# sclaus2/CutFEMx

Measured on AMD Instinct MI355X. Metric: assembled DOFs/sec (active dofs / full hot-path step) + cut-quadrature points/sec, Poisson P1 sphere level-set, higher is better.
Workload: dtype f64; 1 GPU; 3D Poisson P1, sphere level set on 512^3 background mesh (805306368 tets), Nitsche + ghost penalty, runtime quadrature order 4; one step = cut + rules + sparsity + assemble_matrix + assemble_vector + deactivation; cells=805306368, active_dofs=17125633, parallelism=1 gpu

## Files before the change

### cutfemx_amd/csrc/cfx_device.h

```cpp
#pragma once

#include "cfx_common.h"

namespace cfx
{

constexpr int kBlock = 256;
constexpr int kScanItems = 8;
constexpr int kTile = kBlock * kScanItems;

__device__ __forceinline__ int64_t xcd_block_id()
{
  const int64_t per = gridDim.x >> 3;
  return (int64_t)(blockIdx.x & 7) * per + (blockIdx.x >> 3);
}

inline dim3 xcd_grid(int64_t nblocks)
{
  const int64_t g = (nblocks + 7) / 8 * 8;
  if (g > 2147483647LL) throw Error(CFX_ERR_RUNTIME, "grid too large");
  return dim3((unsigned)g);
}

__device__ __forceinline__ void block_fill_run(double* __restrict__ p, int n, double v)
{
  const int head = (int)((reinterpret_cast<uintptr_t>(p) >> 3) & 1) & (n > 0 ? 1 : 0);
  if (threadIdx.x == 0 && head) p[0] = v;
  const int npair = (n - head) >> 1;
  double2* q = reinterpret_cast<double2*>(p + head);
  const double2 vv = make_double2(v, v);
  for (int k = threadIdx.x; k < npair; k += blockDim.x) q[k] = vv;
  if (threadIdx.x == 0 && ((n - head) & 1)) p[n - 1] = v;
}

__host__ __device__ __forceinline__ uint32_t cfx_hash32(uint32_t h)
{
  h ^= h >> 16; h *= 0x85ebca6bu;
  h ^= h >> 13; h *= 0xc2b2ae35u;
  h ^= h >> 16;
  return h;
}

constexpr int kAdjPer = 4, kAdjRun = kBlock * kAdjPer, kAdjSlots = 2 * kAdjRun;
__device__ __forceinline__ int adj_lds_insert(int32_t* s_key, int32_t* s_cnt, int32_t item, int& rank)
{
  unsigned h = cfx_hash32((uint32_t)item) & (kAdjSlots - 1);
  for (;;)
  {
    const int32_t prev = atomicCAS(&s_key[h], -1, item);
    if (prev == -1 || prev == item) break;
    h = (h + 1) & (kAdjSlots - 1);
  }
  rank = atomicAdd(&s_cnt[h], 1);
  return (int)h;
}

template <typename T>
__device__ __forceinline__ T wave_inclusive_scan(T v)
{
  const int lane = threadIdx.x & 63;
#pragma unroll
  for (int d = 1; d < 64; d <<= 1)
  {
    T up = __shfl_up(v, d, 64);
    if (lane >= d) v += up;
  }
  return v;
}

template <typename T>
__device__ __forceinline__ T block_exclusive_scan(T v, T& total)
{
  __shared__ T wave_sums[kBlock / 64];
  const int lane = threadIdx.x & 63, wave = threadIdx.x >> 6;
  T incl = wave_inclusive_scan(v);
  __syncthreads();
  if (lane == 63) wave_sums[wave] = incl;
  __syncthreads();
  T base = 0, tot = 0;
#pragma unroll
  for (int w = 0; w < kBlock / 64; ++w)
  {
    T s = wave_sums[w];
    if (w < wave) base += s;
    tot += s;
  }
  total = tot;
  return base + incl - v;
}

constexpr int kChainLook = 4;
constexpr unsigned long long kScanAggregate = 1ull << 62, kScanPrefix = 2ull << 62, kScanValueMask = (1ull << 62) - 1ull;

struct ChainState
{
  unsigned long long* state = nullptr;
  unsigned int* ticket = nullptr;
};
ChainState chain_state(int64_t ntiles);
inline ChainState fused_chain(bool publish, int64_t ntiles)
{
  const int64_t max_tiles = env_int_once<Sw::FUSED_TILES>(512);
  return publish && ntiles <= max_tiles ? chain_state(ntiles) : ChainState{};
}

__device__ __forceinline__ unsigned int chain_take_tile(unsigned int* __restrict__ ticket)
{
  __shared__ unsigned int s_tile;
  if (threadIdx.x == 0) s_tile = atomicAdd(ticket, 1u);
  __syncthreads();
  return s_tile;
}

__device__ __forceinline__ unsigned long long chain_exclusive_prefix(unsigned long long* __restrict__ state,
                                                                     const unsigned int tile, const unsigned long long total)
// ... 534 lines not shown
```

### cutfemx_amd/csrc/cfx_fem.hip

```cpp
#include <cstdlib>

#include "cfx_elem.h"

using namespace cfx;

namespace
{

struct AsmArgs
{
  const double* x;
  const int32_t* conn;
  const int32_t* dofmap;
  DevN n;
  const int32_t* entities;
  const int32_t* offsets;
  const int32_t* parent_map;
  const double* points;
  const double* weights;
  const double* point_data;
  int point_stride;
  int kernel;
  int qdegree;
  double params[8];
// ... 1114 lines not shown
    }
    return;
  }
  if (!single || !use_rule)
  {
    A.n = single ? 1 : I.n_entities.value();
    A.entities = I.entities.p + (single ? only_index : 0);
    if (A.n.cap > 0)
    {
      if (tdim == 2) launch("assemble_cells2_std", assemble_cells2_kernel<2, false>, grid_for(A.n.cap * nloc0), dim3(kBlock), 0, A, R);
      else launch("assemble_cells2_std", assemble_cells2_kernel<3, false>, grid_for(A.n.cap * nloc0), dim3(kBlock), 0, A, R);
    }
  }
  if (I.rules && (!single || use_rule))
  {
    const cfx_rules_s* Q = I.rules;
    A.n = single ? 1 : Q->nr.value();
    A.offsets = Q->offsets.p + (single ? only_index : 0);
    A.parent_map = Q->parent_map.p + (single ? only_index : 0);
    A.points = Q->points.p; A.weights = Q->weights.p;
    if (A.n.cap > 0)
    {
      if (tdim == 2) launch("assemble_cells2_cut", assemble_cells2_kernel<2, true>, grid_for(A.n.cap * nloc0), dim3(kBlock), 0, A, R);
      else launch("assemble_cells2_cut", assemble_cells2_kernel<3, true>, grid_for(A.n.cap * nloc0), dim3(kBlock), 0, A, R);
    }
  }
}

__global__ void mark_cells_kernel(DevN n_d, const int32_t* __restrict__ cells, int stride, uint8_t* mark)
{
  const int64_t n = dev_n(n_d);
  const int64_t i = (int64_t)blockIdx.x * blockDim.x + threadIdx.x;
  if (i < n) mark[cells[i * stride]] = 1;
}

__global__ void mark_dofs_kernel(int64_t ncells_active, const int32_t* __restrict__ cells,
                                 const int32_t* __restrict__ dofmap, int nd, int bs, uint8_t* indicator)
{
  const int64_t i = (int64_t)blockIdx.x * blockDim.x + threadIdx.x;
  if (i >= ncells_active * nd) return;
  const int64_t c = cells[i / nd];
  const int32_t dof = dofmap[c * nd + (int)(i % nd)];
  for (int k = 0; k < bs; ++k) indicator[(int64_t)dof * bs + k] = 1;
}

bool force_atomic()
{
  return env_equals<Sw::ASSEMBLY>("atomic");
}

struct FlagSet
{
  const uint8_t* f;
  __device__ bool operator()(int64_t i) const { return f[i] != 0; }
};
struct FlagClear
{
  const uint8_t* f;
  __device__ bool operator()(int64_t i) const { return f[i] == 0; }
};

__global__ void deactivate_kernel(DevN n_d, const int32_t* __restrict__ rows, const int64_t* __restrict__ indptr,
                                  const int32_t* __restrict__ indices, double* values, double* b, double diagonal,
                                  double rhs_value, int* error)
{
  const int64_t n = dev_n(n_d);
  const int64_t i = (int64_t)blockIdx.x * blockDim.x + threadIdx.x;
  if (i >= n) return;
  const int32_t r = rows[i];
  if (values)
  {
    const int64_t rb = indptr[r], re = indptr[r + 1];
    const int64_t pos = (re - rb == 1 && indices[rb] == r) ? rb : csr_find(indices, rb, re, r);
    if (pos < 0) *error = 1; else values[pos] = diagonal;
  }
  if (b) b[r] = rhs_value;
}

__global__ void __launch_bounds__(kBlock) deactivate_marks_kernel(int64_t nrows, const uint8_t* __restrict__ rowmark,
                                                                  const int64_t* __restrict__ tile_counts,
                                                                  const int64_t* __restrict__ indptr,
                                                                  const int32_t* __restrict__ indices, double* __restrict__ values,
                                                                  double* __restrict__ b, double diagonal, double rhs_value, int* error,
                                                                  DevN n_active_d, DevN nnz_d)
{
  if (n_active_d.dev && dev_n(n_active_d) == 0) return;
  if (nnz_d.dev && dev_n(nnz_d) == 0) return;
  const int64_t r0 = (int64_t)blockIdx.x * kByteTile;
  const int tl = (int)min((int64_t)kByteTile, nrows - r0);
  const int64_t tc = tile_counts[blockIdx.x];
  const int nact = (int)((tc & 0xffffffffll) + (tc >> 32));
  if (nact == 0 && (!values || indptr[r0 + tl] - indptr[r0] == tl))
  {
    int ok = 1;
    const int64_t e0 = values ? indptr[r0] : 0;
    if (values)
      for (int k = threadIdx.x; k < tl; k += kBlock) ok &= indices[e0 + k] == (int32_t)(r0 + k) ? 1 : 0;
    if (__syncthreads_and(ok))
    {
      if (values) block_fill_run(values + e0, tl, diagonal);
      if (b) block_fill_run(b + r0, tl, rhs_value);
      return;
    }
  }
  if (nact == tl) return;
  for (int k = threadIdx.x; k < tl; k += kBlock)
  {
    const int64_t r = r0 + k;
    if (rowmark[r]) continue;
    if (values)
    {
      const int64_t rb = indptr[r], re = indptr[r + 1];
      const int64_t pos = (re - rb == 1 && indices[rb] == r) ? rb : csr_find(indices, rb, re, (int32_t)r);
      if (pos < 0) *error = 1; else values[pos] = diagonal;
    }
    if (b) b[r] = rhs_value;
  }
}

__global__ void inactive_tile_counts_kernel(int64_t ntiles, int64_t n, const int64_t* __restrict__ active, int32_t* __restrict__ zeros)
{
  const int64_t t = (int64_t)blockIdx.x * blockDim.x + threadIdx.x;
  if (t >= ntiles) return;
  const int64_t len = min((int64_t)kByteTile, n - t * kByteTile);
  zeros[t] = (int32_t)(len - (active[t] & 0xffffffffll) - (active[t] >> 32));
}

__global__ void facet_cells_covered_kernel(DevN nf_d, const int32_t* __restrict__ rows, const uint8_t* __restrict__ cellmark,
                                           int* uncovered)
{
  const int64_t nf = dev_n(nf_d);
  const int64_t i = (int64_t)blockIdx.x * blockDim.x + threadIdx.x;
  if (i >= 2 * nf) return;
  if (cellmark[rows[4 * (i >> 1) + 2 * (i & 1)]] == 0) atomicOr(uncovered, 1);
}

void collect_cell_marks(const cfx_form_s* a, bool include_facets, DevArray<uint8_t>& mark, bool& any)
{
  const int64_t nc = a->V->mesh->ncells;
  mark.alloc(nc);
  mark.zero();
  any = false;
  for (const auto& I : a->integrals)
  {
    if (I.type == CFX_CELL)
    {
      if (I.n_entities.cap() > 0)
      {
        launch("mark_cells", mark_cells_kernel, grid_for(I.n_entities.cap()), dim3(kBlock), 0, I.n_entities, I.entities.p, 1,
               mark.p);
        any = true;
      }
      if (I.rules && I.rules->nr.cap() > 0)
      {
        launch("mark_cells", mark_cells_kernel, grid_for(I.rules->nr.cap()), dim3(kBlock), 0, I.rules->nr,
               I.rules->parent_map.p, 1, mark.p);
        any = true;
      }
    }
    else if (include_facets && I.type == CFX_INTERIOR_FACET && I.n_entities.cap() > 0)
    {
      launch("mark_cells", mark_cells_kernel, grid_for(I.n_entities.cap()), dim3(kBlock), 0, I.n_entities, I.entities.p, 4,
             mark.p);
      launch("mark_cells", mark_cells_kernel, grid_for(I.n_entities.cap()), dim3(kBlock), 0, I.n_entities,
             I.entities.p + 2, 4, mark.p);
      any = true;
    }
  }
}

}

namespace
{
template <int TDIM>
__global__ void __launch_bounds__(kBlock) facet_jump_p1_kernel(DevN n_d, const int32_t* __restrict__ rows,
                                                               const double* __restrict__ x, const int32_t* __restrict__ conn,
                                                               const int32_t* __restrict__ dofmap, double gamma, double hpow,
                                                               int qdegree, double* __restrict__ out, int* error)
{
  const int64_t n = dev_n(n_d);
  constexpr int ND = TDIM + 1;
  const int64_t f = (int64_t)blockIdx.x * kBlock + threadIdx.x;
  if (f >= n) return;
  const int4 row4 = *reinterpret_cast<const int4*>(rows + 4 * f);
  const int64_t c0 = row4.x, c1 = row4.z;
  const int lf0 = row4.y;
  Geo<TDIM> g0, g1;
  load_cell<TDIM>(x, conn, c0, g0);
  load_cell<TDIM>(x, conn, c1, g1);
  jacobian<TDIM>(g0);
  jacobian<TDIM>(g1);
  const double havg = 0.5 * (cell_diameter<TDIM>(g0) + cell_diameter<TDIM>(g1));
  double nrm[TDIM], nn = 0.0;
#pragma unroll
  for (int d = 0; d < TDIM; ++d)
  {
    double v = 0.0;
#pragma unroll
    for (int t = 0; t < TDIM; ++t) v -= g0.K[t][d] * ((lf0 == 0) ? -1.0 : ((lf0 - 1 == t) ? 1.0 : 0.0));
// ... 1230 lines not shown
  cfx_row_plan& plan = *d->plan;
  const int64_t nc = V->mesh->ncells;
  const uint8_t* cell_ind = plan.cellmark.p;
  if (plan.nfacets.value() > 0 && !plan.facet_rows.owned)
  {
    for (const auto& k : plan.key_facets)
      if (k[1] == (int64_t)(uintptr_t)plan.facet_rows.p && k[5] != 0 && dev_block_serial(plan.facet_rows.p) != (uint64_t)k[5])
        throw Error(CFX_ERR_RUNTIME, "stale active domain: the facet list of the form it was made from was released; ask for "
                                     "the lists while the form is alive (the Python wrapper keeps it)");
  }
  if (plan.nfacets.value() > 0)
  {
    ZeroFlag uncovered;
    const int64_t nf = plan.nfacets.value();
    launch("active_cells", facet_cells_covered_kernel, grid_for(nf * 2), dim3(kBlock), 0, nf, plan.facet_rows.p,
           plan.cellmark.p, uncovered.p);
    if (read_scalar(uncovered.p))
    {
      d->cell_indicator.alloc((nc + 3) & ~3LL);
      CFX_HIP(hipMemcpyAsync(d->cell_indicator.p, plan.cellmark.p, (size_t)nc, hipMemcpyDeviceToDevice, ctx().stream));
      launch("mark_cells", mark_cells_kernel, grid_for(nf), dim3(kBlock), 0, nf, plan.facet_rows.p, 4, d->cell_indicator.p);
      launch("mark_cells", mark_cells_kernel, grid_for(nf), dim3(kBlock), 0, nf, plan.facet_rows.p + 2, 4, d->cell_indicator.p);
      cell_ind = d->cell_indicator.p;
    }
  }
  const int32_t* known_tiles = (cell_ind == plan.cellmark.p && plan.cell_tile_counts.n == (nc + kByteTile - 1) / kByteTile)
                                   ? plan.cell_tile_counts.p : nullptr;
  d->n_active = Count(compact_bytes("active_cells", nc, cell_ind, ByteNonZero{}, d->active_cells, known_tiles));
  const int64_t nrows = V->ndofs * V->bs;
  if (V->bs == 1)
    d->n_inactive = Count(compact_bytes("inactive_dofs", nrows, plan.rowmark.p, ByteZero{}, d->inactive_dofs, nullptr,
                                        nrows - plan.n_active_rows.value()));
  else
  {
    DevArray<uint8_t> ind(nrows);
    ind.zero();
    const int64_t nact = d->n_active.value();
    launch("mark_dofs", mark_dofs_kernel, grid_for(nact * V->ndofs_cell), dim3(kBlock), 0, nact,
           d->active_cells.p, V->dofmap.p, V->ndofs_cell, V->bs, ind.p);
    d->n_inactive = Count(compact_bytes("inactive_dofs", nrows, ind.p, ByteZero{}, d->inactive_dofs));
  }
  d->lists_built = true;
}
}

extern "C" {

int cfx_active_view(cfx_active_t d, const int32_t** active_cells, int64_t* n_active, const int32_t** inactive_dofs,
                    int64_t* n_inactive)
{
  CFX_API_BEGIN
  require(d != nullptr, CFX_ERR_INVALID_ARGUMENT, "cfx_active_view: null handle");
  if (!active_cells && !n_active && !inactive_dofs)
  {
    if (n_inactive) *n_inactive = d->V->ndofs * d->V->bs - d->plan->n_active_rows.cap() * d->V->bs;
    return CFX_OK;
  }
  active_lists(d);
  if (active_cells) *active_cells = d->active_cells.p;
  if (n_active) *n_active = d->n_active.cap();
  if (inactive_dofs) *inactive_dofs = d->inactive_dofs.p;
  if (n_inactive) *n_inactive = d->n_inactive.cap();
  CFX_API_END
}

int cfx_deactivate_outside(cfx_active_t d, cfx_pattern_t P, double* values, double* b, double diagonal,
                           double rhs_value)
{
  CFX_API_BEGIN
  require(d && (values == nullptr || P), CFX_ERR_INVALID_ARGUMENT, "cfx_deactivate_outside: null argument");
  const int64_t nrows = d->V->ndofs * d->V->bs;
  std::unique_ptr<OutArray<double>> ov, ob;
  if (values) ov = std::make_unique<OutArray<double>>(values, count_for_buffer(P->nnz, values), true);
  if (b) ob = std::make_unique<OutArray<double>>(b, nrows, true);
  const char* kNoDiag = "Deactivated matrix row has no diagonal entry.";
  ErrorFlag err(CFX_ERR_RUNTIME, kNoDiag);
  cfx_row_plan& plan = *d->plan;
  const int64_t ntiles = (nrows + kByteTile - 1) / kByteTile;
  if (d->V->bs == 1 && plan.row_tile_counts.n == ntiles && (!values || P->nrows == nrows))
  {
    launch("deactivate", deactivate_marks_kernel, dim3((unsigned)ntiles), dim3(kBlock), 0, nrows, plan.rowmark.p,
           plan.row_tile_counts.p, values ? P->indptr.p : (const int64_t*)nullptr, values ? P->indices.p : (const int32_t*)nullptr,
           values ? ov->dev : (double*)nullptr, b ? ob->dev : (double*)nullptr, diagonal, rhs_value, err.p,
           plan.n_active_rows.devn(), values ? P->nnz.devn() : DevN());
  }
  else
  {
    active_lists(d);
    const int64_t n_inactive = d->n_inactive.value();
    if (n_inactive > 0)
      launch("deactivate", deactivate_kernel, grid_for(n_inactive), dim3(kBlock), 0, n_inactive,
             d->inactive_dofs.p, P ? P->indptr.p : nullptr, P ? P->indices.p : nullptr, values ? ov->dev : nullptr,
             b ? ob->dev : nullptr, diagonal, rhs_value, err.p);
  }
  err.check(CFX_ERR_RUNTIME, kNoDiag);
  if (ov) ov->finish();
  if (ob) ob->finish();
  CFX_API_END
}

int cfx_active_destroy(cfx_active_t d)
{
  CFX_API_BEGIN
  delete d;
  CFX_API_END
}

}
```

### cutfemx_amd/csrc/cfx_gather.hip

```cpp
#include <cstdlib>
#include <type_traits>

#include "cfx_elem.h"

using namespace cfx;

namespace cfx
{
void dump_integral(cfx_form_s* a, int integral, int parts, double* out, bool fold_facets = false);
void dump_facet_jumps_p1(cfx_form_s* a, int integral, double* out, int* error);
void dump_facet_jumps_p2(cfx_form_s* a, int integral, int nq, double* out);
void dump_cut_moments(cfx_form_s* a, int integral, double* out);
int quad_npoints(int dim, int degree);
}

namespace
{

constexpr int kWave = 64;
#ifndef CFX_XCD_TILE
#define CFX_XCD_TILE 128
#endif
__device__ __forceinline__ int64_t row_block_id(int64_t b)
{
// ... 2844 lines not shown
        }
    }
    constexpr int W = 2 * NLOC;
    const double* T = A.facet_tensors + f * (int64_t)(W * W);
#pragma unroll
    for (int side = 0; side < 2; ++side)
    {
      double acc[NLOC];
      int csl[ND];
#pragma unroll
      for (int j = 0; j < NLOC; ++j) acc[j] = 0.0;
#pragma unroll
      for (int j = 0; j < ND; ++j) csl[j] = -1;
      if (has)
      {
#pragma unroll
        for (int m = 0; m < 2; ++m)
          if (irow[m] >= 0)
          {
            const double* Tr = T + (int64_t)(irow[m] * BS + kc) * W + side * NLOC;
#pragma unroll
            for (int j = 0; j < NLOC; ++j) acc[j] += Tr[j];
          }
#pragma unroll
        for (int j = 0; j < ND; ++j) csl[j] = find_slot(cols[side][j]);
#pragma unroll
        for (int j = 0; j < ND; ++j)
#pragma unroll
          for (int b = 0; b < BS; ++b)
            if (row_bc || (A.bc1 != nullptr && A.bc1[(int64_t)cols[side][j] * BS + b] != 0)) acc[j * BS + b] = 0.0;
      }
      if constexpr (ORDERED)
      {
        for (int turn = 0; turn < G; ++turn)
        {
          if (gl == turn)
          {
#pragma unroll
            for (int j = 0; j < ND; ++j)
              if (csl[j] >= 0)
              {
#pragma unroll
                for (int b = 0; b < BS; ++b) s_val[grp][csl[j] * BS + b] += acc[j * BS + b];
              }
          }
          __syncthreads();
        }
      }
      else
      {
#pragma unroll
        for (int j = 0; j < ND; ++j)
          if (csl[j] >= 0)
          {
#pragma unroll
            for (int b = 0; b < BS; ++b) atomicAdd(&s_val[grp][csl[j] * BS + b], acc[j * BS + b]);
          }
      }
    }
  }
  __syncthreads();
  if (A.fresh)
    for (int k = gl; k < lene; k += G) A.values[rb + k] = s_val[grp][k];
  else
    for (int k = gl; k < lene; k += G) A.values[rb + k] += s_val[grp][k];
}

__global__ void __launch_bounds__(kBlock) zero_inactive_rows_kernel(int64_t nrows, int bs, const uint8_t* __restrict__ rowmark,
                                                                    const int64_t* __restrict__ indptr, double* __restrict__ values,
                                                                    DevN nnz_d)
{
  const int64_t nnz = dev_n(nnz_d);
  const int64_t R = (int64_t)blockIdx.x * kBlock + threadIdx.x;
  if (R >= nrows || nnz == 0 || rowmark[R / bs]) return;
  const int64_t e1 = min(indptr[R + 1], nnz);
  for (int64_t k = max(indptr[R], (int64_t)0); k < e1; ++k) values[k] = 0.0;
}

__global__ void __launch_bounds__(kBlock) zero_inactive_tiles_kernel(int64_t nrows, const uint8_t* __restrict__ rowmark,
                                                                     const int64_t* __restrict__ tile_counts,
                                                                     const int64_t* __restrict__ indptr, double* __restrict__ values,
                                                                     DevN nnz_d)
{
  const int64_t nnz = dev_n(nnz_d);
  if (nnz == 0) return;
  const int64_t r0 = (int64_t)blockIdx.x * kByteTile;
  const int n = (int)min((int64_t)kByteTile, nrows - r0);
  if (tile_counts[blockIdx.x] == 0)
  {
    const int64_t e0 = indptr[r0];
    if (e0 >= 0 && e0 + n <= nnz) block_fill_run(values + e0, n, 0.0);
    return;
  }
  for (int k = threadIdx.x; k < n; k += kBlock)
    if (!rowmark[r0 + k])
    {
      const int64_t e1 = min(indptr[r0 + k + 1], nnz);
      for (int64_t e = max(indptr[r0 + k], (int64_t)0); e < e1; ++e) values[e] = 0.0;
    }
}

template <int TDIM, int DEG, int G>
__global__ void __launch_bounds__(kWave) assemble_vec_rows_kernel(RowArgs A)
{
  constexpr int ND = Elem<TDIM, DEG>::ND;
  constexpr int RPW = kWave / G;
  const int lane = threadIdx.x, grp = lane / G, gl = lane % G;
  const int64_t ri = CFX_ROW_BLOCK * RPW + grp;
  if (A.vec_skip && dev_n(A.vec_n_odd) == 0) return;
  bool live = ri < dev_n(A.n_active) && A.cellmark != nullptr;
  const int64_t r = live ? A.active_rows[ri] : 0;
  if (live && A.vec_skip && A.vec_skip[r] > 0) live = false;
  const int64_t cb = live ? A.d2c_off[r] : 0;
  const int nc = live ? (int)(A.d2c_off[r + 1] - cb) : 0;
  double part = 0.0;
  const unsigned dpos = (live && A.slot4) ? (A.diagpos[r] & kDiagPosMask) : 0u;
  constexpr int R = G <= 4 ? 6 : 4;
  for (int base = 0;; base += R * G)
  {
    if (__ballot(base + gl < nc) == 0) break;
    int64_t cell[R];
    uint8_t mk[R];
    int lr[R];
    uint32_t s4[R];
#pragma unroll
    for (int k = 0; k < R; ++k)
    {
      const int t = base + k * G + gl;
      cell[k] = t < nc ? (int64_t)A.d2c[cb + t] : -1;
      s4[k] = (A.slot4 && t < nc) ? A.slot4[cb + t] : 0u;
      if (DEG == 2 && A.slotn && t < nc) s4[k] = reinterpret_cast<const uint32_t*>(A.slotn + (cb + t) * 12)[2];
    }
#pragma unroll
    for (int k = 0; k < R; ++k) mk[k] = cell[k] >= 0 ? A.cellmark[cell[k]] : (uint8_t)0;
#pragma unroll
    for (int k = 0; k < R; ++k)
    {
      lr[k] = 0;
      if (!mk[k]) continue;
      if (DEG == 2 && A.slotn) lr[k] = (int)((s4[k] >> 16) & 0xffu);
      else if (A.slot4)
      {
#pragma unroll
        for (int j = 0; j < ND; ++j) lr[k] = (((s4[k] >> (8 * j)) & 0xffu) == dpos) ? j : lr[k];
      }
      else
      {
#pragma unroll
        for (int j = 0; j < ND; ++j) lr[k] = (A.dofmap[cell[k] * ND + j] == (int32_t)r) ? j : lr[k];
      }
    }
#pragma unroll
    for (int k = 0; k < R; ++k)
    {
      if (!mk[k]) continue;
      const int64_t c = cell[k];
      for (int i = 0; i < A.n_cell; ++i)
      {
        const RowIntegral& I = A.cell[i];
        if ((mk[k] & (1u << i)) && I.std_tensors)
          part += I.std_tensors[(int64_t)lr[k] * I.n_std + (I.std_by_cell ? c : entity_index(I.std_bits, I.std_rank, c))];
        if (mk[k] & (16u << i))
          for (int64_t e = first_rule(I.rule_keys, I.rule_first, I.rule_mask, (int32_t)c); e < dev_len(I.nr) && I.parent_map[e] == c; ++e)
            part += I.rule_tensors[e * ND + lr[k]];
      }
    }
  }
#pragma unroll
  for (int d = G / 2; d >= 1; d >>= 1) part += __shfl_xor(part, d, G);
  if (live && gl == 0) A.values[r] += part;
}

bool deterministic()
{
  return env_is<Sw::DETERMINISTIC>('1');
}

struct P2PlainArgs
{
  int64_t n;
  const int32_t* rows;
  const double* x;
// ... 2051 lines not shown
```

### cutfemx_amd/csrc/cfx_rowasm.hip

```cpp
#include <cmath>
#include <cstdlib>


#include "cfx_elem.h"

using namespace cfx;

namespace
{

constexpr int kWave = 64;

__global__ void plan_mark_cells_kernel(DevN n_d, const int32_t* __restrict__ cells, int stride, uint8_t bit,
                                       uint8_t* mark)
{
  const int64_t n = dev_n(n_d);
  const int64_t i = (int64_t)blockIdx.x * blockDim.x + threadIdx.x;
  if (i >= n) return;
  const int64_t c = cells[i * stride];
  mark[c] = mark[c] | bit;
}

__global__ void __launch_bounds__(kBlock) plan_pack_bits_kernel(int64_t ncells, const uint8_t* __restrict__ mark, uint8_t bit,
                                                                unsigned long long* __restrict__ words,
// ... 916 lines not shown
        const int4 q4 = l4[m];
        rank += (q4.x < v ? 1 : 0) + (q4.y < v ? 1 : 0) + (q4.z < v ? 1 : 0) + (q4.w < v ? 1 : 0);
      }
      if (P.indices)
      {
        const int bc = P.bs_col ? P.bs_col : P.bs;
        for (int a = 0; a < P.bs; ++a)
          for (int b = 0; b < bc; ++b)
            P.indices[P.indptr[r * P.bs + a] + (int64_t)rank * bc + b] = v * bc + b;
      }
      else
        P.tmp[ri * T + rank] = v;
    }
  if (cnt >= T) *P.overflow = 1;
  if (live && gl == 0 && !P.indices)
  {
    if (cnt > *reinterpret_cast<volatile int*>(P.maxlen)) atomicMax(P.maxlen, cnt);
    P.len[ri] = cnt;
    for (int a = 0; a < P.bs; ++a) P.counts[r * P.bs + a] = cnt * (P.bs_col ? P.bs_col : P.bs);
  }
  __syncthreads();
  }
}

__global__ void fill_i32_kernel(int64_t n, int32_t v, int32_t* out)
{
  const int64_t i = (int64_t)blockIdx.x * blockDim.x + threadIdx.x;
  if (i < n) out[i] = v;
}

__global__ void pattern_diag_kernel(int64_t ndofs, int bs, const uint8_t* __restrict__ rowmark,
                                    const int64_t* __restrict__ indptr, int32_t* __restrict__ indices)
{
  const int64_t r = (int64_t)blockIdx.x * blockDim.x + threadIdx.x;
  if (r >= ndofs || rowmark[r]) return;
  for (int a = 0; a < bs; ++a)
    for (int b = 0; b < bs; ++b) indices[indptr[r * bs + a] + b] = (int32_t)(r * bs + b);
}

__global__ void __launch_bounds__(kBlock) indptr_reduce_kernel(int64_t nrows, int bs, const uint8_t* __restrict__ rowmark,
                                                               const int32_t* __restrict__ counts, int64_t* __restrict__ tile_sums)
{
  const int64_t tile = (int64_t)blockIdx.x * kTile;
  int64_t s = 0;
  if (bs == 1 && tile + kTile <= nrows)
  {
    static_assert(kScanItems == 8, "eight rows per thread");
    const int64_t r0 = tile + 8 * threadIdx.x;
    const uint2 m = *reinterpret_cast<const uint2*>(rowmark + r0);
    if ((m.x | m.y) == 0u) s = 8;
    else
    {
#pragma unroll
      for (int q = 0; q < 8; ++q)
      {
        const unsigned byte = ((q < 4 ? m.x : m.y) >> (8 * (q & 3))) & 0xffu;
        s += byte ? counts[r0 + q] : 1;
      }
    }
  }
  else
  {
#pragma unroll
    for (int k = 0; k < kScanItems; ++k)
    {
      const int64_t R = tile + k * kBlock + threadIdx.x;
      if (R < nrows) s += rowmark[R / bs] ? counts[R] : bs;
    }
  }
  int64_t total;
  (void)block_exclusive_scan<int64_t>(s, total);
  if (threadIdx.x == 0) tile_sums[blockIdx.x] = total;
}

template <typename First>
__device__ __forceinline__ int64_t indptr_tile(int64_t nrows, int bs, const uint8_t* __restrict__ rowmark,
                                               const int32_t* __restrict__ counts, const int64_t tile, First first,
                                               int64_t* __restrict__ indptr, int32_t* __restrict__ indices,
                                               const int64_t nnz_cap)
{
  __shared__ int64_t s_v[kTile];
  if (bs == 1 && tile + kTile <= nrows)
  {
    static_assert(kScanItems == 8, "eight rows per thread");
    const uint2 m = *reinterpret_cast<const uint2*>(rowmark + tile + 8 * threadIdx.x);
    if (__syncthreads_or((m.x | m.y) != 0u) == 0)
    {
      const int64_t t0 = first((int64_t)kTile);
      const int64_t p0 = t0 + 8 * threadIdx.x;
      const int64_t r0 = tile + 8 * threadIdx.x;
      if ((reinterpret_cast<uintptr_t>(indptr + r0) & 15) == 0)
      {
        longlong2* ip = reinterpret_cast<longlong2*>(indptr + r0);
#pragma unroll
        for (int q = 0; q < 4; ++q) ip[q] = make_longlong2(p0 + 2 * q, p0 + 2 * q + 1);
      }
      else
      {
#pragma unroll
        for (int q = 0; q < 8; ++q) indptr[r0 + q] = p0 + q;
      }
      if (p0 >= 0 && p0 + 8 <= nnz_cap)
      {
#pragma unroll
        for (int q = 0; q < 8; ++q) indices[p0 + q] = (int32_t)(r0 + q);
      }
      else
      {
        for (int q = 0; q < 8; ++q)
          if (p0 + q >= 0 && p0 + q + 1 <= nnz_cap) indices[p0 + q] = (int32_t)(r0 + q);
      }
      return t0 + kTile;
    }
  }
#pragma unroll
  for (int k = 0; k < kScanItems; ++k)
  {
    const int i = k * kBlock + threadIdx.x;
    const int64_t R = tile + i;
    s_v[i] = R < nrows ? (rowmark[R / bs] ? (int64_t)counts[R] : (int64_t)bs) : 0;
  }
  __syncthreads();
  int64_t v[kScanItems], s = 0;
#pragma unroll
  for (int k = 0; k < kScanItems; ++k) { v[k] = s_v[threadIdx.x * kScanItems + k]; s += v[k]; }
  int64_t total;
  const int64_t local = block_exclusive_scan<int64_t>(s, total);
  const int64_t t0 = first(total);
  int64_t off = local + t0;
#pragma unroll
  for (int k = 0; k < kScanItems; ++k) { s_v[threadIdx.x * kScanItems + k] = off; off += v[k]; }
  __syncthreads();
#pragma unroll
  for (int k = 0; k < kScanItems; ++k)
  {
    const int i = k * kBlock + threadIdx.x;
    const int64_t R = tile + i;
    if (R >= nrows) continue;
    const int64_t p = s_v[i];
    indptr[R] = p;
    const int64_t dof = R / bs;
    if (!rowmark[dof] && p >= 0 && p + bs <= nnz_cap)
      for (int b = 0; b < bs; ++b) indices[p + b] = (int32_t)(dof * bs + b);
  }
  return t0 + total;
}

__global__ void __launch_bounds__(kBlock) indptr_write_kernel(int64_t nrows, int bs, const uint8_t* __restrict__ rowmark,
                                                              const int32_t* __restrict__ counts,
                                                              const int64_t* __restrict__ tile_offsets,
                                                              int64_t* __restrict__ indptr, int32_t* __restrict__ indices,
                                                              DevN nnz_d)
{
  const int64_t nnz_cap = nnz_d.dev ? dev_n(nnz_d) : INT64_MAX;
  const int64_t end = indptr_tile(nrows, bs, rowmark, counts, (int64_t)blockIdx.x * kTile,
                                  [&](int64_t) { return tile_offsets[blockIdx.x]; }, indptr, indices, nnz_cap);
  if (blockIdx.x == gridDim.x - 1 && threadIdx.x == kBlock - 1) indptr[nrows] = end;
}

__global__ void __launch_bounds__(kBlock) indptr_chained_kernel(int64_t nrows, int bs, const uint8_t* __restrict__ rowmark,
                                                                const int32_t* __restrict__ counts,
                                                                int64_t* __restrict__ indptr, int32_t* __restrict__ indices,
                                                                int64_t nnz_cap, ChainState chain,
                                                                int64_t* __restrict__ total_out, CountJobs after)
{
  const unsigned int tile = chain_take_tile(chain.ticket);
  const int64_t end = indptr_tile(nrows, bs, rowmark, counts, (int64_t)tile * kTile,
                                  [&](int64_t total) { return (int64_t)chain_exclusive_prefix(chain.state, tile, (unsigned long long)total); },
                                  indptr, indices, nnz_cap);
  if (tile == gridDim.x - 1 && threadIdx.x == kBlock - 1)
  {
    indptr[nrows] = end;
    *total_out = end;
    if (after.n > 0) count_publish(after);
  }
}

template <int T>
__global__ void pattern_write_kernel(DevN n_active_d, const int32_t* __restrict__ active_rows, int bs,
                                     const int32_t* __restrict__ tmp, const int32_t* __restrict__ len,
                                     const int64_t* __restrict__ indptr, int32_t* __restrict__ indices)
{
  const int64_t n_active = dev_n(n_active_d);
  const int64_t i = (int64_t)blockIdx.x * blockDim.x + threadIdx.x;
  const int64_t ri = i / 8;
  if (ri >= n_active) return;
  const int n = len[ri];
  const int64_t r = active_rows ? (int64_t)active_rows[ri] : ri;
  if (bs == 1)
  {
    const int4* src = reinterpret_cast<const int4*>(tmp + ri * T);
    const int64_t ob = indptr[r];
    for (int k4 = (int)(i - ri * 8); 4 * k4 < n; k4 += 8)
    {
      const int4 v = src[k4];
      const int k = 4 * k4;
// ... 2930 lines not shown
```

Measured before the change: 1.254 billion DOF/s.

## Vectorize inactive-row handling per wavefront using ballot-detected contiguous row runs

Replaces per-tile all-or-nothing inactive handling in deactivation, value zeroing and indptr/indices construction with a per-wavefront scheme. It ballots 16-row groups that are fully inactive and merges them into contiguous runs, then fills those runs with wide vector stores, falling back to per-row work only for mixed groups. Partially active tiles near the level-set surface get coalesced stores instead of scattered per-row ones. The deactivation kernel also skips checking the diagonal pattern when the pattern was built from the same plan. The cost is more complex wave-level control flow with shuffles and ballots, and it depends on the fixed tile/group sizes set by the static_asserts.

```diff
diff --git a/cutfemx_amd/csrc/cfx_device.h b/cutfemx_amd/csrc/cfx_device.h
--- a/cutfemx_amd/csrc/cfx_device.h
+++ b/cutfemx_amd/csrc/cfx_device.h
@@ -22,15 +22,111 @@
   return dim3((unsigned)g);
 }
 
-__device__ __forceinline__ void block_fill_run(double* __restrict__ p, int n, double v)
+__device__ __forceinline__ void fill_run(double* __restrict__ p, int64_t n, double v, int t, int nt)
 {
   const int head = (int)((reinterpret_cast<uintptr_t>(p) >> 3) & 1) & (n > 0 ? 1 : 0);
-  if (threadIdx.x == 0 && head) p[0] = v;
-  const int npair = (n - head) >> 1;
+  if (t == 0 && head) p[0] = v;
+  const int64_t npair = (n - head) >> 1;
   double2* q = reinterpret_cast<double2*>(p + head);
   const double2 vv = make_double2(v, v);
-  for (int k = threadIdx.x; k < npair; k += blockDim.x) q[k] = vv;
-  if (threadIdx.x == 0 && ((n - head) & 1)) p[n - 1] = v;
+  for (int64_t k = t; k < npair; k += nt) q[k] = vv;
+  if (t == 0 && ((n - head) & 1)) p[n - 1] = v;
+}
+__device__ __forceinline__ void iota_run(int32_t* __restrict__ p, int n, int32_t v0, int t, int nt)
+{
+  const int head = min(n, (int)((0u - (unsigned)(reinterpret_cast<uintptr_t>(p) >> 2)) & 3u));
+  if (t < head) p[t] = v0 + t;
+  const int nquad = (n - head) >> 2;
+  int4* q = reinterpret_cast<int4*>(p + head);
+  for (int k = t; k < nquad; k += nt)
+  {
+    const int32_t v = v0 + head + 4 * k;
+    q[k] = make_int4(v, v + 1, v + 2, v + 3);
+  }
+  const int done = head + 4 * nquad;
+  if (t < n - done) p[done + t] = v0 + done + t;
+}
+__device__ __forceinline__ bool iota_run_holds(const int32_t* __restrict__ p, int n, int32_t v0, int t, int nt)
+{
+  const int head = min(n, (int)((0u - (unsigned)(reinterpret_cast<uintptr_t>(p) >> 2)) & 3u));
+  bool ok = t >= head || p[t] == v0 + t;
+  const int nquad = (n - head) >> 2;
+  const int4* q = reinterpret_cast<const int4*>(p + head);
+  for (int k = t; k < nquad; k += nt)
+  {
+    const int32_t v = v0 + head + 4 * k;
+    const int4 w = q[k];
+    ok = ok && w.x == v && w.y == v + 1 && w.z == v + 2 && w.w == v + 3;
+  }
+  const int done = head + 4 * nquad;
+  return ok && (t >= n - done || p[done + t] == v0 + done + t);
+}
+
+__device__ __forceinline__ bool take_bit_run(unsigned long long& mask, int& first, int& count)
+{
+  if (mask == 0ull) return false;
+  first = __ffsll((long long)mask) - 1;
+  const unsigned long long rest = ~(mask >> first);
+  count = rest ? __ffsll((long long)rest) - 1 : 64;
+  mask &= ~((count == 64 ? ~0ull : (1ull << count) - 1ull) << first);
+  return true;
+}
+
+constexpr int kGroupRows = 16, kWaveGroupRows = 64 * kGroupRows;
+template <typename Run, typename Row>
+__device__ __forceinline__ void wave_inactive_rows(const uint8_t* __restrict__ rowmark, const int64_t* __restrict__ indptr,
+                                                   int64_t w0, int64_t nrows, bool none_marked, Run run, Row row)
+{
+  const int lane = threadIdx.x & 63;
+  const int64_t g0 = w0 + (int64_t)kGroupRows * lane;
+  bool uniform = false, mixed = false;
+  uint4 m = make_uint4(~0u, ~0u, ~0u, ~0u);
+  if (g0 + kGroupRows <= nrows)
+  {
+    if (none_marked) uniform = true;
+    else
+    {
+      m = *reinterpret_cast<const uint4*>(rowmark + g0);
+      uniform = (m.x | m.y | m.z | m.w) == 0u;
+      auto zero_byte = [](unsigned w) { return ((w - 0x01010101u) & ~w & 0x80808080u) != 0u; };
+      mixed = !uniform && (zero_byte(m.x) || zero_byte(m.y) || zero_byte(m.z) || zero_byte(m.w));
+    }
+  }
+  else if (g0 < nrows)
+  {
+    mixed = true;
+    unsigned w[4] = {~0u, ~0u, ~0u, ~0u};
+    for (int k = 0; k < (int)(nrows - g0); ++k)
+      if (rowmark[g0 + k] == 0) w[k >> 2] &= ~(0xffu << (8 * (k & 3)));
+    m = make_uint4(w[0], w[1], w[2], w[3]);
+  }
+  const unsigned long long all_runs = __ballot(uniform);
+  int64_t e_lo = 0, e_hi = 0;
+  if (indptr && uniform)
+  {
+    if (lane == 0 || ((all_runs >> (lane - 1)) & 1ull) == 0ull) e_lo = indptr[g0];
+    if (lane == 63 || ((all_runs >> (lane + 1)) & 1ull) == 0ull) e_hi = indptr[g0 + kGroupRows];
+  }
+  unsigned long long runs = all_runs;
+  int first, count;
+  while (take_bit_run(runs, first, count))
+    run(w0 + (int64_t)kGroupRows * first, kGroupRows * count, __shfl(e_lo, first, 64), __shfl(e_hi, first + count - 1, 64));
+  unsigned long long rest = __ballot(mixed);
+  while (rest)
+  {
+    int g = -1;
+#pragma unroll
+    for (int q = 0; q < 64 / kGroupRows; ++q)
+      if (rest)
+      {
+        if (lane / kGroupRows == q) g = __ffsll((long long)rest) - 1;
+        rest &= rest - 1ull;
+      }
+    const int src = g < 0 ? lane : g, k = lane % kGroupRows;
+    const unsigned wx = __shfl(m.x, src, 64), wy = __shfl(m.y, src, 64), wz = __shfl(m.z, src, 64), ww = __shfl(m.w, src, 64);
+    const unsigned word = k < 8 ? (k < 4 ? wx : wy) : (k < 12 ? wz : ww);
+    if (g >= 0 && ((word >> (8 * (k & 3))) & 0xffu) == 0u) row(w0 + (int64_t)kGroupRows * g + k);
+  }
 }
 
 __host__ __device__ __forceinline__ uint32_t cfx_hash32(uint32_t h)
diff --git a/cutfemx_amd/csrc/cfx_fem.hip b/cutfemx_amd/csrc/cfx_fem.hip
--- a/cutfemx_amd/csrc/cfx_fem.hip
+++ b/cutfemx_amd/csrc/cfx_fem.hip
@@ -1220,32 +1220,17 @@
                                                                   const int64_t* __restrict__ indptr,
                                                                   const int32_t* __restrict__ indices, double* __restrict__ values,
                                                                   double* __restrict__ b, double diagonal, double rhs_value, int* error,
-                                                                  DevN n_active_d, DevN nnz_d)
+                                                                  DevN n_active_d, DevN nnz_d, bool own_pattern)
 {
   if (n_active_d.dev && dev_n(n_active_d) == 0) return;
   if (nnz_d.dev && dev_n(nnz_d) == 0) return;
-  const int64_t r0 = (int64_t)blockIdx.x * kByteTile;
-  const int tl = (int)min((int64_t)kByteTile, nrows - r0);
-  const int64_t tc = tile_counts[blockIdx.x];
-  const int nact = (int)((tc & 0xffffffffll) + (tc >> 32));
-  if (nact == 0 && (!values || indptr[r0 + tl] - indptr[r0] == tl))
-  {
-    int ok = 1;
-    const int64_t e0 = values ? indptr[r0] : 0;
-    if (values)
-      for (int k = threadIdx.x; k < tl; k += kBlock) ok &= indices[e0 + k] == (int32_t)(r0 + k) ? 1 : 0;
-    if (__syncthreads_and(ok))
-    {
-      if (values) block_fill_run(values + e0, tl, diagonal);
-      if (b) block_fill_run(b + r0, tl, rhs_value);
-      return;
-    }
-  }
-  if (nact == tl) return;
-  for (int k = threadIdx.x; k < tl; k += kBlock)
-  {
-    const int64_t r = r0 + k;
-    if (rowmark[r]) continue;
+  static_assert(kByteTile == (kBlock / 64) * kWaveGroupRows, "a wavefront's groups per quarter of the tile");
+  const int64_t nnz = values ? dev_n(nnz_d) : 0;
+  const int64_t w0 = (int64_t)blockIdx.x * kByteTile + (int64_t)kWaveGroupRows * (threadIdx.x >> 6);
+  if (w0 >= nrows) return;
+  const int lane = threadIdx.x & 63;
+  auto one_row = [&](int64_t r)
+  {
     if (values)
     {
       const int64_t rb = indptr[r], re = indptr[r + 1];
@@ -1253,7 +1238,25 @@
       if (pos < 0) *error = 1; else values[pos] = diagonal;
     }
     if (b) b[r] = rhs_value;
-  }
+  };
+  wave_inactive_rows(
+      rowmark, values ? indptr : (const int64_t*)nullptr, w0, nrows, tile_counts[blockIdx.x] == 0,
+      [&](int64_t r, int n, int64_t e0, int64_t e1)
+      {
+        if (values)
+        {
+          bool diag = e0 >= 0 && e0 + n <= nnz && e1 - e0 == n;
+          if (diag && !own_pattern) diag = __all(iota_run_holds(indices + e0, n, (int32_t)r, lane, 64)) != 0;
+          if (!diag)
+          {
+            for (int k = lane; k < n; k += 64) one_row(r + k);
+            return;
+          }
+          fill_run(values + e0, n, diagonal, lane, 64);
+        }
+        if (b) fill_run(b + r, n, rhs_value, lane, 64);
+      },
+      one_row);
 }
 
 __global__ void inactive_tile_counts_kernel(int64_t ntiles, int64_t n, const int64_t* __restrict__ active, int32_t* __restrict__ zeros)
@@ -2650,7 +2653,7 @@
     launch("deactivate", deactivate_marks_kernel, dim3((unsigned)ntiles), dim3(kBlock), 0, nrows, plan.rowmark.p,
            plan.row_tile_counts.p, values ? P->indptr.p : (const int64_t*)nullptr, values ? P->indices.p : (const int32_t*)nullptr,
            values ? ov->dev : (double*)nullptr, b ? ob->dev : (double*)nullptr, diagonal, rhs_value, err.p,
-           plan.n_active_rows.devn(), values ? P->nnz.devn() : DevN());
+           plan.n_active_rows.devn(), values ? P->nnz.devn() : DevN(), values && P->built_plan == plan.serial);
   }
   else
   {
diff --git a/cutfemx_amd/csrc/cfx_gather.hip b/cutfemx_amd/csrc/cfx_gather.hip
--- a/cutfemx_amd/csrc/cfx_gather.hip
+++ b/cutfemx_amd/csrc/cfx_gather.hip
@@ -2950,22 +2950,24 @@
                                                                      const int64_t* __restrict__ indptr, double* __restrict__ values,
                                                                      DevN nnz_d)
 {
+  static_assert(kByteTile == (kBlock / 64) * kWaveGroupRows, "a wavefront's groups per quarter of the tile");
   const int64_t nnz = dev_n(nnz_d);
   if (nnz == 0) return;
-  const int64_t r0 = (int64_t)blockIdx.x * kByteTile;
-  const int n = (int)min((int64_t)kByteTile, nrows - r0);
-  if (tile_counts[blockIdx.x] == 0)
-  {
-    const int64_t e0 = indptr[r0];
-    if (e0 >= 0 && e0 + n <= nnz) block_fill_run(values + e0, n, 0.0);
-    return;
-  }
-  for (int k = threadIdx.x; k < n; k += kBlock)
-    if (!rowmark[r0 + k])
-    {
-      const int64_t e1 = min(indptr[r0 + k + 1], nnz);
-      for (int64_t e = max(indptr[r0 + k], (int64_t)0); e < e1; ++e) values[e] = 0.0;
-    }
+  const int64_t w0 = (int64_t)blockIdx.x * kByteTile + (int64_t)kWaveGroupRows * (threadIdx.x >> 6);
+  if (w0 >= nrows) return;
+  const int lane = threadIdx.x & 63;
+  wave_inactive_rows(
+      rowmark, indptr, w0, nrows, tile_counts[blockIdx.x] == 0,
+      [&](int64_t, int, int64_t p0, int64_t p1)
+      {
+        const int64_t e0 = max(p0, (int64_t)0), e1 = min(p1, nnz);
+        if (e0 < e1) fill_run(values + e0, e1 - e0, 0.0, lane, 64);
+      },
+      [&](int64_t r)
+      {
+        const int64_t e1 = min(indptr[r + 1], nnz);
+        for (int64_t e = max(indptr[r], (int64_t)0); e < e1; ++e) values[e] = 0.0;
+      });
 }
 
 template <int TDIM, int DEG, int G>
diff --git a/cutfemx_amd/csrc/cfx_rowasm.hip b/cutfemx_amd/csrc/cfx_rowasm.hip
--- a/cutfemx_amd/csrc/cfx_rowasm.hip
+++ b/cutfemx_amd/csrc/cfx_rowasm.hip
@@ -1022,36 +1022,84 @@
   __shared__ int64_t s_v[kTile];
   if (bs == 1 && tile + kTile <= nrows)
   {
-    static_assert(kScanItems == 8, "eight rows per thread");
-    const uint2 m = *reinterpret_cast<const uint2*>(rowmark + tile + 8 * threadIdx.x);
-    if (__syncthreads_or((m.x | m.y) != 0u) == 0)
+    static_assert(kScanItems == 8 && 2 * kScanItems == kGroupRows, "eight rows per thread, a 16-row group per lane pair");
+    const int64_t r0 = tile + 8 * threadIdx.x;
+    const uint2 m = *reinterpret_cast<const uint2*>(rowmark + r0);
+    const bool none = (m.x | m.y) == 0u;
+    auto diag_run = [&](int64_t p, int64_t r, int n, int t, int nt)
+    {
+      const int64_t lo = max(p, (int64_t)0), hi = min(p + n, nnz_cap);
+      if (lo < hi) iota_run(indices + lo, (int)(hi - lo), (int32_t)(r + (lo - p)), t, nt);
+    };
+    const bool wide = (reinterpret_cast<uintptr_t>(indptr + tile) & 15) == 0;
+    auto indptr_out = [&](auto value)
+    {
+      if (wide)
+      {
+        longlong2* ip = reinterpret_cast<longlong2*>(indptr + tile);
+#pragma unroll
+        for (int k = 0; k < kScanItems / 2; ++k)
+        {
+          const int i = k * kBlock + threadIdx.x;
+          ip[i] = make_longlong2(value(2 * i), value(2 * i + 1));
+        }
+      }
+      else
+      {
+#pragma unroll
+        for (int k = 0; k < kScanItems; ++k) indptr[tile + k * kBlock + threadIdx.x] = value(k * kBlock + threadIdx.x);
+      }
+    };
+    if (__syncthreads_or(!none) == 0)
     {
       const int64_t t0 = first((int64_t)kTile);
-      const int64_t p0 = t0 + 8 * threadIdx.x;
-      const int64_t r0 = tile + 8 * threadIdx.x;
-      if ((reinterpret_cast<uintptr_t>(indptr + r0) & 15) == 0)
-      {
-        longlong2* ip = reinterpret_cast<longlong2*>(indptr + r0);
-#pragma unroll
-        for (int q = 0; q < 4; ++q) ip[q] = make_longlong2(p0 + 2 * q, p0 + 2 * q + 1);
-      }
-      else
-      {
-#pragma unroll
-        for (int q = 0; q < 8; ++q) indptr[r0 + q] = p0 + q;
-      }
-      if (p0 >= 0 && p0 + 8 <= nnz_cap)
-      {
-#pragma unroll
-        for (int q = 0; q < 8; ++q) indices[p0 + q] = (int32_t)(r0 + q);
-      }
-      else
-      {
-        for (int q = 0; q < 8; ++q)
-          if (p0 + q >= 0 && p0 + q + 1 <= nnz_cap) indices[p0 + q] = (int32_t)(r0 + q);
-      }
+      indptr_out([&](int i) { return t0 + i; });
+      diag_run(t0, tile, kTile, threadIdx.x, kBlock);
       return t0 + kTile;
     }
+    int64_t v[kScanItems], s = 0;
+    {
+      int4 c0 = make_int4(1, 1, 1, 1), c1 = c0;
+      if (!none)
+      {
+        c0 = reinterpret_cast<const int4*>(counts + r0)[0];
+        c1 = reinterpret_cast<const int4*>(counts + r0)[1];
+      }
+      const int c[kScanItems] = {c0.x, c0.y, c0.z, c0.w, c1.x, c1.y, c1.z, c1.w};
+#pragma unroll
+      for (int q = 0; q < kScanItems; ++q)
+      {
+        v[q] = (((q < 4 ? m.x : m.y) >> (8 * (q & 3))) & 0xffu) ? (int64_t)c[q] : 1;
+        s += v[q];
+      }
+    }
+    int64_t total;
+    const int64_t local = block_exclusive_scan<int64_t>(s, total);
+    const int64_t t0 = first(total);
+    const int64_t p0 = local + t0;
+    {
+      int64_t off = p0;
+#pragma unroll
+      for (int q = 0; q < kScanItems; ++q) { s_v[threadIdx.x * kScanItems + q] = off; off += v[q]; }
+    }
+    __syncthreads();
+    indptr_out([&](int i) { return s_v[i]; });
+    const int lane = threadIdx.x & 63;
+    const bool uniform = none && __shfl_xor((int)none, 1, 64) != 0;
+    unsigned long long runs = __ballot(uniform);
+    int f, c;
+    while (take_bit_run(runs, f, c)) diag_run(__shfl(p0, f, 64), r0 + 8 * (f - lane), 8 * c, lane, 64);
+    if (!uniform)
+    {
+      int64_t p = p0;
+#pragma unroll
+      for (int q = 0; q < kScanItems; ++q)
+      {
+        if ((((q < 4 ? m.x : m.y) >> (8 * (q & 3))) & 0xffu) == 0u && p >= 0 && p < nnz_cap) indices[p] = (int32_t)(r0 + q);
+        p += v[q];
+      }
+    }
+    return t0 + total;
   }
 #pragma unroll
   for (int k = 0; k < kScanItems; ++k)
```

Result: faster. 1.314 billion DOF/s, median of 6 (+4.9%).
